# stecrotti/MPSKit.jl

Hardware: AMD Instinct MI355X
Metric: DMRG sweeps/sec + ddAC matvec achieved-TFLOP/s, Heisenberg L=100 D=1024 fp64 (higher is better)
Workload: dtype f64; 1 GPU; Heisenberg S=1/2 FiniteMPS L=100 D=1024 d=2 W=5 fp64, 1-site DMRG sweep (2L-2 site updates), fixed Krylov budget 8 matvecs/site; parallelism=single GPU

## Files before the change

include/mpsk.h:

```cpp
#ifndef MPSK_H
#define MPSK_H
#include <stddef.h>
#include <stdint.h>

#ifdef __cplusplus
extern "C" {
#endif

typedef struct mpsk_ctx mpsk_ctx;
typedef struct mpsk_mposlice mpsk_mposlice;

enum { MPSK_F64 = 0, MPSK_C128 = 1 };
enum { MPSK_OK = 0, MPSK_ERR_INVALID = 1, MPSK_ERR_HIP = 2, MPSK_ERR_UNSUPPORTED = 3, MPSK_ERR_NOMEM = 4 };
enum { MPSK_BLOCK_ZERO = 0, MPSK_BLOCK_SCALAR = 1, MPSK_BLOCK_DENSE = 2 };

int mpsk_version(void);
const char* mpsk_last_error(void);

int mpsk_ctx_create(int device, mpsk_ctx** out);
int mpsk_ctx_destroy(mpsk_ctx* ctx);
int mpsk_ctx_set_stream(mpsk_ctx* ctx, void* hip_stream);
int mpsk_ctx_set_dtype(mpsk_ctx* ctx, int dtype);
int mpsk_ctx_get_stream(mpsk_ctx* ctx, void** hip_stream);
int mpsk_ctx_get_device(mpsk_ctx* ctx, int* device);
// ... 39 lines not shown
int mpsk_hac_destroy(mpsk_hac* h);
int mpsk_hac_info(const mpsk_hac* h, int* mode, int* nslabs);
int mpsk_dC(mpsk_ctx* ctx, int W, int Dlo, int Dl, int Dr, const void* GL, const void* GR,
            const void* c, void* y);
int mpsk_dAC2(mpsk_ctx* ctx, const mpsk_mposlice* H1, const mpsk_mposlice* H2, int Dlo, int Dl, int Dr,
              const void* GL, const void* GR, const void* x2, void* y2);

int mpsk_dAC_proj(mpsk_ctx* ctx, const mpsk_mposlice* H, int Dlo, int Dl, int Dr, int Dro, const void* GL, const void* GR,
                  const void* x, void* y);
int mpsk_dAC2_proj(mpsk_ctx* ctx, const mpsk_mposlice* H1, const mpsk_mposlice* H2, int Dlo, int Dl, int Dm, int Dr, int Dro,
                   const void* GL, const void* GR, const void* AC, const void* AR, void* Y);

int mpsk_dAC2_product(mpsk_ctx* ctx, const mpsk_mposlice* H1, const mpsk_mposlice* H2, int Dl, int Dm, int Dr,
                      const void* GL, const void* GR, const void* AC, const void* AR, void* Y);
int mpsk_complement_tsvd(mpsk_ctx* ctx, int m, int n, const void* Y, int ldy, const void* QL, int ldql, int pl,
                         const void* QR, int ldqr, int pr, int k, void* U, int ldu, void* S, void* Vt, int ldvt, int* kept);
int mpsk_ctx_complement_stats(mpsk_ctx* ctx, long* n_calls, long* n_subspace, long* n_full);

int mpsk_transfer_left(mpsk_ctx* ctx, const mpsk_mposlice* H, int W, int d, int Dl, int Dr, int Dlb,
                       int Drb, const void* GLin, const void* A, const void* Ab, void* GLout);
int mpsk_transfer_right(mpsk_ctx* ctx, const mpsk_mposlice* H, int W, int d, int Dl, int Dr, int Dlb,
                        int Drb, const void* A, const void* Ab, const void* GRin, void* GRout);
enum { MPSK_TRANSFER_CANONICAL = 1 };
int mpsk_transfer_left_ex(mpsk_ctx* ctx, const mpsk_mposlice* H, int W, int d, int Dl, int Dr, int Dlb, int Drb,
                          const void* GLin, const void* A, const void* Ab, int flags, void* GLout);
int mpsk_transfer_right_ex(mpsk_ctx* ctx, const mpsk_mposlice* H, int W, int d, int Dl, int Dr, int Dlb, int Drb,
                           const void* A, const void* Ab, const void* GRin, int flags, void* GRout);
int mpsk_regularize(mpsk_ctx* ctx, int W, int D1, int D2, void* v, const void* lvec, const void* rvec);

int mpsk_qrpos(mpsk_ctx* ctx, int m, int n, const void* A, int lda, void* Q, int ldq, void* R, int ldr);
int mpsk_qrpos2(mpsk_ctx* ctx, int m, int n, const void* A1, int lda1, void* Q1, int ldq1, void* R1, int ldr1,
                const void* A2, int lda2, void* Q2, int ldq2, void* R2, int ldr2);
int mpsk_qrlq_pair(mpsk_ctx* ctx, int m, int n, const void* A1, int lda1, void* Q1, int ldq1, void* R1, int ldr1,
                   const void* A2, int lda2, void* L2, int ldl2, void* Q2, int ldq2);
int mpsk_lqpos(mpsk_ctx* ctx, int m, int n, const void* A, int lda, void* L, int ldl, void* Q, int ldq);
int mpsk_ctx_qr_defer(mpsk_ctx* ctx);
int mpsk_ctx_side_mark(mpsk_ctx* ctx);
int mpsk_ctx_side_begin(mpsk_ctx* ctx);
int mpsk_ctx_side_end(mpsk_ctx* ctx);
int mpsk_qr_commit(mpsk_ctx* ctx, int* redone);
int mpsk_tsvd(mpsk_ctx* ctx, int m, int n, const void* theta, int ldt, void* U, int ldu, void* S, void* Vh,
              int ldv, int max_keep, double trunc_err, int* kept, double* disc_norm);
int mpsk_tsplit(mpsk_ctx* ctx, int m, int n, const void* theta, int ldt, int max_keep, double trunc_err,
                void* AL, int ldal, void* C, int ldc, void* AR, int ldar, void* S, int* kept, double* disc_norm);
int mpsk_cx_embed(mpsk_ctx* ctx, int m, int n, const void* H, int64_t ldh, void* E, int64_t lde);
int mpsk_cx_half(mpsk_ctx* ctx, int m, int n, const void* E, int64_t lde, void* H, int64_t ldh);
// ... 40 lines not shown
```

mpskit.jl_amd/_lib.py:

```python
from __future__ import annotations

import ctypes as C
import os

_HERE = os.path.dirname(os.path.abspath(__file__))
LIB_PATH = os.environ.get("MPSK_LIB") or os.path.join(_HERE, "libmpsk.so")


class MpskError(RuntimeError):
    pass


_lib = None

c_void_pp = C.POINTER(C.c_void_p)
c_int32_p = C.POINTER(C.c_int32)
c_double_p = C.POINTER(C.c_double)

SIGNATURES = {
    "mpsk_ctx_create": [C.c_int, c_void_pp],
    "mpsk_ctx_destroy": [C.c_void_p],
    "mpsk_ctx_set_stream": [C.c_void_p, C.c_void_p],
    "mpsk_ctx_synchronize": [C.c_void_p],
    "mpsk_ctx_workspace_reserve": [C.c_void_p, C.c_size_t],
# ... 32 lines not shown
    "mpsk_dAC2": [C.c_void_p, C.c_void_p, C.c_void_p, C.c_int, C.c_int, C.c_int, C.c_void_p, C.c_void_p,
                  C.c_void_p, C.c_void_p],
    "mpsk_transfer_left": [C.c_void_p, C.c_void_p, C.c_int, C.c_int, C.c_int, C.c_int, C.c_int, C.c_int,
                           C.c_void_p, C.c_void_p, C.c_void_p, C.c_void_p],
    "mpsk_transfer_right": [C.c_void_p, C.c_void_p, C.c_int, C.c_int, C.c_int, C.c_int, C.c_int, C.c_int,
                            C.c_void_p, C.c_void_p, C.c_void_p, C.c_void_p],
    "mpsk_transfer_left_ex": [C.c_void_p, C.c_void_p, C.c_int, C.c_int, C.c_int, C.c_int, C.c_int, C.c_int,
                              C.c_void_p, C.c_void_p, C.c_void_p, C.c_int, C.c_void_p],
    "mpsk_transfer_right_ex": [C.c_void_p, C.c_void_p, C.c_int, C.c_int, C.c_int, C.c_int, C.c_int, C.c_int,
                               C.c_void_p, C.c_void_p, C.c_void_p, C.c_int, C.c_void_p],
    "mpsk_regularize": [C.c_void_p, C.c_int, C.c_int, C.c_int, C.c_void_p, C.c_void_p, C.c_void_p],
    "mpsk_qrpos": [C.c_void_p, C.c_int, C.c_int, C.c_void_p, C.c_int, C.c_void_p, C.c_int, C.c_void_p, C.c_int],
    "mpsk_qrpos2": [C.c_void_p, C.c_int, C.c_int, C.c_void_p, C.c_int, C.c_void_p, C.c_int, C.c_void_p, C.c_int,
                    C.c_void_p, C.c_int, C.c_void_p, C.c_int, C.c_void_p, C.c_int],
    "mpsk_qrlq_pair": [C.c_void_p, C.c_int, C.c_int, C.c_void_p, C.c_int, C.c_void_p, C.c_int, C.c_void_p, C.c_int,
                       C.c_void_p, C.c_int, C.c_void_p, C.c_int, C.c_void_p, C.c_int],
    "mpsk_lqpos": [C.c_void_p, C.c_int, C.c_int, C.c_void_p, C.c_int, C.c_void_p, C.c_int, C.c_void_p, C.c_int],
    "mpsk_tsvd": [C.c_void_p, C.c_int, C.c_int, C.c_void_p, C.c_int, C.c_void_p, C.c_int, C.c_void_p,
                  C.c_void_p, C.c_int, C.c_int, C.c_double, C.POINTER(C.c_int), c_double_p],
    "mpsk_tsplit": [C.c_void_p, C.c_int, C.c_int, C.c_void_p, C.c_int, C.c_int, C.c_double, C.c_void_p, C.c_int,
                    C.c_void_p, C.c_int, C.c_void_p, C.c_int, C.c_void_p, C.POINTER(C.c_int), c_double_p],
    "mpsk_gemm": [C.c_void_p, C.c_int, C.c_int, C.c_int, C.c_int, C.c_int, C.c_double, C.c_void_p,
                  C.c_int64, C.c_void_p, C.c_int64, C.c_double, C.c_void_p, C.c_int64],
    "mpsk_copy2d": [C.c_void_p, C.c_int, C.c_int, C.c_void_p, C.c_int64, C.c_void_p, C.c_int64],
    "mpsk_vdot": [C.c_void_p, C.c_int64, C.c_void_p, C.c_void_p, c_double_p],
    "mpsk_vnrm2": [C.c_void_p, C.c_int64, C.c_void_p, c_double_p],
    "mpsk_vaxpby": [C.c_void_p, C.c_int64, C.c_double, C.c_void_p, C.c_double, C.c_void_p],
    "mpsk_vscal": [C.c_void_p, C.c_int64, C.c_double, C.c_void_p],
    "mpsk_vtimes_i": [C.c_void_p, C.c_int64, C.c_void_p, C.c_void_p],
    "mpsk_vcopy": [C.c_void_p, C.c_int64, C.c_void_p, C.c_void_p],
    "mpsk_vzero": [C.c_void_p, C.c_int64, C.c_void_p],
    "mpsk_vmultidot": [C.c_void_p, C.c_int64, C.c_int, c_void_pp, C.c_void_p, c_double_p],
    "mpsk_vgs_step": [C.c_void_p, C.c_int64, C.c_int, c_void_pp, C.c_void_p, c_double_p],
    "mpsk_vorth_step": [C.c_void_p, C.c_int64, C.c_int, c_void_pp, C.c_void_p, c_double_p, c_double_p],
    "mpsk_vorth_step_dev": [C.c_void_p, C.c_int64, C.c_int, c_void_pp, C.c_void_p, C.c_void_p],
    "mpsk_vlincomb": [C.c_void_p, C.c_int64, C.c_int, c_void_pp, c_double_p, C.c_void_p],
    "mpsk_cx_embed": [C.c_void_p, C.c_int, C.c_int, C.c_void_p, C.c_int64, C.c_void_p, C.c_int64],
    "mpsk_cx_half": [C.c_void_p, C.c_int, C.c_int, C.c_void_p, C.c_int64, C.c_void_p, C.c_int64],
    "mpsk_vmultilincomb": [C.c_void_p, C.c_int64, C.c_int, c_void_pp, C.c_int, c_void_pp, c_double_p],
    "mpsk_vnormalize_dev": [C.c_void_p, C.c_int64, C.c_void_p, C.c_void_p, C.c_void_p],
    "mpsk_vnrm2_dev": [C.c_void_p, C.c_int64, C.c_void_p, C.c_void_p],
    "mpsk_ctx_qr_retries": [C.c_void_p, C.POINTER(C.c_long)],
    "mpsk_ctx_qr_defer": [C.c_void_p],
    "mpsk_ctx_side_mark": [C.c_void_p],
    "mpsk_ctx_side_begin": [C.c_void_p],
    "mpsk_ctx_side_end": [C.c_void_p],
# ... 96 lines not shown
```

mpskit.jl_amd/csrc/mpsk_api.hip:

```cpp
#include <hip/hip_runtime.h>
#include <cstdio>
#include <cstdlib>
#include <cstring>
#include <cmath>
#include <algorithm>
#include <map>
#include <string>
#include <vector>
#include "mpsk.h"
#include "mpsk_internal.h"

using namespace mpsk;

static thread_local std::string g_err;
static int fail(int code, const std::string& msg) { g_err = msg; return code; }
#define HIPCHK(expr)                                                                        \
  do {                                                                                      \
    hipError_t e_ = (expr);                                                                 \
    if (e_ != hipSuccess)                                                                   \
      return fail(MPSK_ERR_HIP, std::string(#expr) + ": " + hipGetErrorString(e_));         \
  } while (0)
#define REQUIRE(cond, msg)                                                  \
  do {                                                                      \
    if (!(cond)) return fail(MPSK_ERR_INVALID, std::string(__func__) + ": " + (msg)); \
  } while (0)

static constexpr int MPSK_DENSE_MIN_CHID = 8;

struct mpsk_mposlice {
  mpsk_ctx* ctx;
  int Wl, Wr, d;
  int dtype = MPSK_F64;
  std::vector<double> Ofull;
  std::vector<double> Ofull_im;
  MixPlan fwd;
  MixPlan bwd;
  MixPlan rgt;
  double Oi(int w, int t, int s, int v) const {
    return Ofull_im.empty() ? 0.0 : Ofull_im[w + (size_t)Wl * (t + d * (s + (size_t)d * v))];
  }
  std::vector<char> row_used, col_used;
  MixPlan rc;
  std::vector<int> rc_w, rc_s, rc_t;
  int rc_nseg = 0;
  bool jordan = false;
  MixPlan jr, jl;
  std::vector<int> jr_p, jl_p;
  int jr_nseg = 0, jl_nseg = 0;
  MixPlan tl, tr;
  bool tl_dblock = false;
  mutable std::map<int64_t, int64_t*> jtabL;
  mutable std::map<std::pair<int64_t, int64_t>, int64_t*> jtabR;
  double O(int w, int t, int s, int v) const { return Ofull[w + (size_t)Wl * (t + d * (s + (size_t)d * v))]; }
  bool dense = false;
  double* d_Od = nullptr;
  mutable std::map<std::pair<int64_t, int64_t>, int64_t*> dtab;
  double* d_OdR = nullptr;
  mutable std::map<std::pair<int64_t, int64_t>, int64_t*> dtabR;
};

struct PoolBuf { void* p; size_t bytes; bool used; hipStream_t last = nullptr; hipEvent_t ev = nullptr; bool ev_set = false; };

struct mpsk_ctx {
  int device = 0;
  hipStream_t stream = nullptr;
  void* ws = nullptr;
  size_t ws_bytes = 0;
  double* d_scal = nullptr;
  double* d_partial = nullptr;
  double* h_scal = nullptr;
  double* d_coef = nullptr;
  double* h_coef = nullptr;
  hipEvent_t ev_coef = nullptr;
// ... 347 lines not shown
        }
        out.assign((size_t)d * nseg, empty);
        for (int t = 0; t < d; ++t) {
          int k = 0;
          for (int si = 0; si < d; ++si) if (used[si + d * t]) out[(size_t)t * nseg + k++] = si + d * t;
        }
      };
      lists(r_used, s->jr_p, s->jr_nseg);
      lists(l_used, s->jl_p, s->jl_nseg);
      HIPCHK(mix_plan_create(jr, d * d, Wr, &s->jr));
      HIPCHK(mix_plan_create(jl, d * d, Wl, &s->jl));
      s->jordan = s->jr_nseg > 0 && s->jl_nseg > 0;
      if (s->jordan && !cx) {
        std::vector<MixTerm> tl, tr;
        for (int t = 0; t < d; ++t)
          for (int si = 0; si < d; ++si) {
            for (int v = 1; v < Wr; ++v)
              if (s->O(0, t, si, v) != 0.0) { tl.push_back({t + d * (v - 1), si, s->O(0, t, si, v)}); if (v == Wr - 1) s->tl_dblock = true; }
            for (int w = 1; w < Wl - 1; ++w)
              if (s->O(w, t, si, Wr - 1) != 0.0) tr.push_back({t + d * (w - 1), si, s->O(w, t, si, Wr - 1)});
          }
        HIPCHK(mix_plan_create(tl, d * (Wr - (s->tl_dblock ? 1 : 2)), d, &s->tl));
        HIPCHK(mix_plan_create(tr, d * (Wl - 2), d, &s->tr));
      }
    }
  }
  if (dense) {
    const int Wl = s->Wl, Wr = s->Wr;
    std::vector<double> od((size_t)d * Wl * d * Wr);
    for (int v = 0; v < Wr; ++v)
      for (int t = 0; t < d; ++t)
        for (int w = 0; w < Wl; ++w)
          for (int si = 0; si < d; ++si)
            od[(si + (size_t)d * w) + (size_t)d * Wl * (t + (size_t)d * v)] = s->O(w, t, si, v);
    s->dense = true;
    if (hipMalloc(&s->d_Od, sizeof(double) * od.size()) != hipSuccess) { mpsk_mposlice_destroy(s); return fail(MPSK_ERR_NOMEM, "dense MPO hipMalloc failed"); }
    HIPCHK(hipMemcpy(s->d_Od, od.data(), sizeof(double) * od.size(), hipMemcpyHostToDevice));
    for (int v = 0; v < Wr; ++v)
      for (int t = 0; t < d; ++t)
        for (int w = 0; w < Wl; ++w)
          for (int si = 0; si < d; ++si)
            od[(si + (size_t)d * v) + (size_t)d * Wr * (t + (size_t)d * w)] = s->O(w, t, si, v);
    if (hipMalloc(&s->d_OdR, sizeof(double) * od.size()) != hipSuccess) { mpsk_mposlice_destroy(s); return fail(MPSK_ERR_NOMEM, "dense MPO hipMalloc failed"); }
    HIPCHK(hipMemcpy(s->d_OdR, od.data(), sizeof(double) * od.size(), hipMemcpyHostToDevice));
  }
  *out = s;
// ... 15 lines not shown
  const void* blocks[1] = {O};
  return mposlice_build(c, dtype, 1, &cl, &cr, d, &kind, nullptr, blocks, true, out);
}

int mpsk_mposlice_destroy(mpsk_mposlice* s) {
  if (!s) return MPSK_OK;
  mpsk_ctx* c = s->ctx;
  (void)hipSetDevice(c->device);
  (void)hipStreamSynchronize(c->stream);
  for (auto it = c->pair_plans.begin(); it != c->pair_plans.end();) {
    if (it->first.first == s || it->first.second == s) { mix_plan_destroy(&it->second); it = c->pair_plans.erase(it); }
    else ++it;
  }
  mix_plan_destroy(&s->fwd);
  mix_plan_destroy(&s->bwd);
  mix_plan_destroy(&s->rgt);
  mix_plan_destroy(&s->rc);
  mix_plan_destroy(&s->jr);
  mix_plan_destroy(&s->jl);
  mix_plan_destroy(&s->tl);
  mix_plan_destroy(&s->tr);
  for (auto& kv : s->jtabL) (void)hipFree(kv.second);
  for (auto& kv : s->jtabR) (void)hipFree(kv.second);
  if (s->d_Od) (void)hipFree(s->d_Od);
  if (s->d_OdR) (void)hipFree(s->d_OdR);
  for (auto& kv : s->dtab) (void)hipFree(kv.second);
  for (auto& kv : s->dtabR) (void)hipFree(kv.second);
  delete s;
  return MPSK_OK;
}

int mpsk_mposlice_dims(const mpsk_mposlice* s, int* Wl, int* Wr, int* d) {
  REQUIRE(s, "slice is NULL");
  if (Wl) *Wl = s->Wl;
  if (Wr) *Wr = s->Wr;
  if (d) *d = s->d;
  return MPSK_OK;
}

}

static int ensure_ws(mpsk_ctx* c, size_t bytes) {
  if (c->pend.active) return fail(MPSK_ERR_INVALID, "a deferred factorization still owns the workspace: call mpsk_qr_commit first");
  if (c->on_side) return fail(MPSK_ERR_INVALID, "workspace users are not accepted on the side stream: call mpsk_ctx_side_end first");
  if (bytes <= c->ws_bytes) return MPSK_OK;
  return mpsk_ctx_workspace_reserve(c, bytes + bytes / 4);
}

static GemmArgs mk(const double* A, const double* B, double* C, int M, int N, int K, int64_t lda, int64_t ldb,
                   int64_t ldc, int tA = 0, int tB = 0) {
  GemmArgs g;
// ... 823 lines not shown
  if (left) { auto it = H->jtabL.find(Dl); if (it != H->jtabL.end()) { *out = it->second; return MPSK_OK; } }
  else { auto it = H->jtabR.find({Dl, Dr}); if (it != H->jtabR.end()) { *out = it->second; return MPSK_OK; } }
  const int d = H->d, n = left ? H->jl_nseg : H->jr_nseg;
  const std::vector<int>& plist = left ? H->jl_p : H->jr_p;
  const int64_t tL = (int64_t)Dl * d * Dl, tR = (int64_t)Dr * d * Dr;
  std::vector<int64_t> h((size_t)2 * d * n);
  for (int t = 0; t < d; ++t)
    for (int k = 0; k < n; ++k) {
      const int p = plist[(size_t)t * n + k], si = p % d, tt = p / d;
      if (left) { h[(size_t)t * n + k] = tt * tL + (int64_t)si * Dl; h[(size_t)(d + t) * n + k] = (int64_t)si * Dl; }
      else { h[(size_t)t * n + k] = (int64_t)si * Dl; h[(size_t)(d + t) * n + k] = tt * tR + (int64_t)si * Dr; }
    }
  int64_t* p = nullptr;
  if (hipMalloc(&p, sizeof(int64_t) * h.size()) != hipSuccess) return fail(MPSK_ERR_NOMEM, "transfer segment table hipMalloc failed");
  if (hipMemcpy(p, h.data(), sizeof(int64_t) * h.size(), hipMemcpyHostToDevice) != hipSuccess) {
    (void)hipFree(p);
    return fail(MPSK_ERR_HIP, "transfer segment table upload failed");
  }
  if (left) H->jtabL.emplace(Dl, p); else H->jtabR.emplace(std::make_pair((int64_t)Dl, (int64_t)Dr), p);
  *out = p;
  return MPSK_OK;
}

static int transfer_left_canonical(mpsk_ctx* c, const mpsk_mposlice* H, int Dl, int Dr, const double* GLin, const double* A,
                                   double* GLout) {
  const int d = H->d, Wr = H->Wr, n2 = H->jl_nseg;
  if (hac_check_on())
    if (int rc = transfer_canonical_check(c, "mpsk_transfer_left_ex", GLin, Dl, A, d, Dl, Dr, true)) return rc;
  const size_t slab = (size_t)Dl * d * Dr;
  const int64_t tL = (int64_t)Dl * d * Dl;
  const size_t nL = up32((size_t)d * tL);
  if (int rc = ensure_ws(c, sizeof(double) * (nL + slab * (Wr - 1)))) return rc;
  const int64_t* tab = nullptr;
  if (int rc = jordan_tab(H, true, Dl, Dr, &tab)) return rc;
  double* GLc = (double*)c->ws;
  double* T2 = GLc + nL;
  double* T = T2 + slab * (Wr - 2);
  SlabIndex il{1 << 30, 1, (int64_t)Dl * Dl, 0, 0, (int64_t)Dl}, ol{d, 1 << 30, (int64_t)Dl, tL, 0, (int64_t)d * Dl};
  HIPCHK(mix_apply(H->jl, GLin, il, GLc, ol, Dl, Dl, c->stream));
  SlabIndex ia{1 << 30, 1, (int64_t)Dl, 0, 0, (int64_t)Dl * d}, ot{d, 1 << 30, (int64_t)Dl, (int64_t)slab, 0, (int64_t)Dl * d};
  HIPCHK(mix_apply(H->tl, A, ia, T2, ot, Dl, Dr, c->stream));
  GemmArgs g = mk(GLc, A, T, Dl, Dr, Dl, (int64_t)Dl * d, (int64_t)Dl * d, (int64_t)Dl * d);
  g.batch = d; g.bsA = 0; g.bsB = 0; g.bsC = (int64_t)Dl;
  g.beta = H->tl_dblock ? 1.0 : 0.0;
  g.nseg = n2; g.zsegA = tab; g.zsegB = tab + (size_t)d * n2;
  g.tabs_even = Dl % 2 == 0;
  g.tag = 1;
  HIPCHK(gemm_f64(g, c->stream));
  HIPCHK(identity_slab(GLout, Dr, c->stream));
  GemmArgs g3 = mk(A, T2, GLout + (size_t)Dr * Dr, Dr, Dr, Dl * d, (int64_t)Dl * d, (int64_t)Dl * d, Dr, 1, 0);
  g3.batch = Wr - 1; g3.bsA = 0; g3.bsB = (int64_t)slab; g3.bsC = (int64_t)Dr * Dr;
  HIPCHK(gemm_f64(g3, c->stream));
  return MPSK_OK;
}

static int transfer_right_canonical(mpsk_ctx* c, const mpsk_mposlice* H, int Dl, int Dr, const double* A, const double* GRin,
                                    double* GRout) {
  const int d = H->d, Wl = H->Wl, Wr = H->Wr, n1 = H->jr_nseg;
  if (hac_check_on())
    if (int rc = transfer_canonical_check(c, "mpsk_transfer_right_ex", GRin + (size_t)(Wr - 1) * Dr * Dr, Dr, A, d, Dl, Dr, false))
      return rc;
  const size_t slab = (size_t)Dl * d * Dr;
  const int64_t tR = (int64_t)Dr * d * Dr;
  const size_t nR = up32((size_t)d * tR);
  if (int rc = ensure_ws(c, sizeof(double) * (nR + slab * (Wl - 1)))) return rc;
  const int64_t* tab = nullptr;
  if (int rc = jordan_tab(H, false, Dl, Dr, &tab)) return rc;
  double* GRc = (double*)c->ws;
  double* X = GRc + nR;
  SlabIndex ir{1 << 30, 1, (int64_t)Dr * Dr, 0, 0, (int64_t)Dr}, orr{d, 1 << 30, (int64_t)Dr, tR, 0, (int64_t)d * Dr};
  HIPCHK(mix_apply(H->jr, GRin, ir, GRc, orr, Dr, Dr, c->stream));
  SlabIndex ia{1 << 30, 1, (int64_t)Dl, 0, 0, (int64_t)Dl * d}, ox{d, 1 << 30, (int64_t)Dl, (int64_t)slab, 0, (int64_t)Dl * d};
  HIPCHK(mix_apply(H->tr, A, ia, X + slab, ox, Dl, Dr, c->stream));
  GemmArgs g = mk(A, GRc, X, Dl, Dr, Dr, (int64_t)Dl * d, (int64_t)Dr * d, (int64_t)Dl * d);
  g.batch = d; g.bsA = 0; g.bsB = 0; g.bsC = (int64_t)Dl;
  g.nseg = n1; g.zsegA = tab; g.zsegB = tab + (size_t)d * n1;
  g.tabs_even = Dl % 2 == 0 && Dr % 2 == 0;
  g.tag = 1;
  HIPCHK(gemm_f64(g, c->stream));
  HIPCHK(identity_slab(GRout + (size_t)(Wl - 1) * Dl * Dl, Dl, c->stream));
  std::vector<int64_t> sa;
  for (int t = 0; t < d; ++t) sa.push_back((int64_t)t * Dl);
  GemmArgs g3 = mk(X, A, GRout, Dl, Dl, Dr, (int64_t)Dl * d, (int64_t)Dl * d, Dl, 0, 1);
  g3.batch = Wl - 1; g3.bsA = (int64_t)slab; g3.bsB = 0; g3.bsC = (int64_t)Dl * Dl;
  HIPCHK(gemm_segments(g3, sa, sa, c->stream));
  return MPSK_OK;
}

int mpsk_transfer_left_ex(mpsk_ctx* c, const mpsk_mposlice* H, int W, int d, int Dl, int Dr, int Dlb, int Drb,
                          const void* GLin, const void* A, const void* Ab, int flags, void* GLout) {
  REQUIRE(c && GLin && A && Ab && GLout, "NULL argument");
  REQUIRE((flags & ~MPSK_TRANSFER_CANONICAL) == 0, "unknown flags");
  if (transfer_canonical_ok(H, flags, A, Ab, Dl, Dr, Dlb, Drb)) {
    REQUIRE(Dl > 0 && Dr > 0, "dimensions must be positive");
    HIPCHK(hipSetDevice(c->device));
    return transfer_left_canonical(c, H, Dl, Dr, (const double*)GLin, (const double*)A, (double*)GLout);
  }
  return mpsk_transfer_left(c, H, W, d, Dl, Dr, Dlb, Drb, GLin, A, Ab, GLout);
}

int mpsk_transfer_right_ex(mpsk_ctx* c, const mpsk_mposlice* H, int W, int d, int Dl, int Dr, int Dlb, int Drb,
                           const void* A, const void* Ab, const void* GRin, int flags, void* GRout) {
  REQUIRE(c && GRin && A && Ab && GRout, "NULL argument");
  REQUIRE((flags & ~MPSK_TRANSFER_CANONICAL) == 0, "unknown flags");
  if (transfer_canonical_ok(H, flags, A, Ab, Dl, Dr, Dlb, Drb)) {
    REQUIRE(Dl > 0 && Dr > 0, "dimensions must be positive");
    HIPCHK(hipSetDevice(c->device));
// ... 1710 lines not shown
```

mpskit.jl_amd/csrc/mpsk_gemm.hip:

```cpp
#include <hip/hip_runtime.h>
#include <stdint.h>
#include <cstdio>
#include <cstdlib>
#include <map>
#include <mutex>
#include <string>
#include <vector>
#include "mpsk_internal.h"

namespace mpsk {

typedef double d4 __attribute__((ext_vector_type(4)));
typedef double d2 __attribute__((ext_vector_type(2)));

constexpr int BK = 16;
constexpr int NTHREADS = 256;

template <int BMN, bool KMAJOR> struct LdsImg {
  static_assert(BK == 16, "the K-major swizzle assumes 128-byte rows");
  static constexpr int STRIDE = KMAJOR ? BK : (BMN + 16);
  static constexpr int SIZE = KMAJOR ? BMN * BK : BK * (BMN + 16);
  __device__ static inline int idx(int mn, int k) { return KMAJOR ? mn * BK + (k ^ (mn & 15)) : k * STRIDE + mn; }
};

// ... 378 lines not shown
  const int ntiles = tilesM * tilesN;
  int bid = blockIdx.x;
  if (!g.xcd_interleave) {
    int q = ntiles / 8, r = ntiles % 8, xcd = bid % 8, pos = bid / 8;
    bid = (xcd < r ? xcd * (q + 1) : r * (q + 1) + (xcd - r) * q) + pos;
  }
  int bm, bn;
  tile_coords(g, bid, tilesM, tilesN, &bm, &bn);
  if (g.upper_only && bm > bn) return;
  const int z = blockIdx.y;
  const int m0 = bm * BM, n0 = bn * BN;
  const double* Ab = g.A + (g.tabA ? g.tabA[z] : (int64_t)z * g.bsA);
  const double* Bb = g.B + (g.tabB ? g.tabB[z] : (int64_t)z * g.bsB);
  double* Cb = g.C + (g.tabC ? g.tabC[z] : (int64_t)z * g.bsC);
  d4 acc[BM / 32][BN / 32];
#pragma unroll
  for (int i = 0; i < BM / 32; ++i)
#pragma unroll
    for (int j = 0; j < BN / 32; ++j) acc[i][j] = d4{0.0, 0.0, 0.0, 0.0};
  const int nt = ((g.K + BK - 1) / BK) * g.nseg;
  int ktlo = 0, kthi = nt;
  if (g.b_upper) { const int lim = (n0 + BN + BK - 1) / BK; if (lim < kthi) kthi = lim; }
  if (g.a_upper) ktlo = m0 / BK;
  if (ktlo < kthi) gemm_acc_dispatch<BM, BN, TA, TB, ALIGNED, ZS, CJ>(g, Ab, Bb, z, m0, n0, ktlo, kthi, acc, smem);
  gemm_store_c<BM, BN, ALIGNED, CJ>(g, Cb, z, m0, n0, acc);
}

template <int BM, int BN, bool TA, bool TB, bool ALIGNED, bool ZS = false>
__device__ __forceinline__ void gemm_sk_body(const GemmArgs& g) {
  extern __shared__ __attribute__((aligned(16))) double smem[];
  constexpr int WTM = BM / 2, WTN = BN / 2, TM = WTM / 16, TN = WTN / 16;
  const int tilesM = (g.M + BM - 1) / BM, tilesN = (g.N + BN - 1) / BN;
  const int ntiles = tilesM * tilesN;
  const int KT = ((g.K + BK - 1) / BK) * g.nseg;
  const int U = ntiles * g.batch * KT;
  int sid = blockIdx.x;
  if (!g.xcd_interleave) {
    const int nwg = gridDim.x;
    int q = nwg / 8, r = nwg % 8, xcd = sid % 8, pos = sid / 8;
    sid = (xcd < r ? xcd * (q + 1) : r * (q + 1) + (xcd - r) * q) + pos;
  }
  int u = sid * g.sk_units;
  int slot = sid;
  if (g.sk_split_major) {
    const int TZ = ntiles * g.batch;
    const int split = sid / TZ, tzs = sid - split * TZ;
// ... 3 lines not shown
  const int uend = (u + g.sk_units < U) ? u + g.sk_units : U;
  const int lane = threadIdx.x & 63, wave = threadIdx.x >> 6;
  const int wm = wave & 1, wn = wave >> 1, fr = lane & 15, fq = lane >> 4;
  while (u < uend) {
    const int tz = u / KT;
    const int kt0 = u - tz * KT;
    const int kt1 = (uend - u < KT - kt0) ? kt0 + (uend - u) : KT;
    const int z = tz / ntiles, tile = tz - z * ntiles;
    int bm, bn;
    tile_coords(g, tile, tilesM, tilesN, &bm, &bn);
    if (g.upper_only && bm > bn) { u += kt1 - kt0; continue; }
    const int m0 = bm * BM, n0 = bn * BN;
    const double* Ab = g.A + (g.tabA ? g.tabA[z] : (int64_t)z * g.bsA);
    const double* Bb = g.B + (g.tabB ? g.tabB[z] : (int64_t)z * g.bsB);
    d4 acc[TM][TN];
#pragma unroll
    for (int i = 0; i < TM; ++i)
#pragma unroll
      for (int j = 0; j < TN; ++j) acc[i][j] = d4{0.0, 0.0, 0.0, 0.0};
    {
      int ka = kt0, kb = kt1;
      if (g.b_upper) { const int lim = (n0 + BN + BK - 1) / BK; if (lim < kb) kb = lim; }
      if (g.a_upper) { const int lo = m0 / BK; if (lo > ka) ka = lo; }
      if (ka < kb) gemm_acc_dispatch<BM, BN, TA, TB, ALIGNED, ZS, false>(g, Ab, Bb, z, m0, n0, ka, kb, acc, smem);
    }
    const bool toC = (kt0 == 0);
    double* base = toC ? g.C + (g.tabC ? g.tabC[z] : (int64_t)z * g.bsC) + m0 + (int64_t)n0 * g.ldc
                       : g.sk_ws + (int64_t)slot * BM * BN;
    const int64_t ld = toC ? g.ldc : BM;
    const double beta = toC ? g.beta : 0.0;
    const double alpha = g.alpha;
    const int mlim = toC ? g.M - m0 : BM, nlim = toC ? g.N - n0 : BN;
    const bool split = toC && g.tabC2 != nullptr;
#pragma unroll
    for (int i = 0; i < TM; ++i) {
      const int m = wm * WTM + i * 16 + fr;
#pragma unroll
      for (int j = 0; j < TN; ++j) {
#pragma unroll
        for (int rg = 0; rg < 4; ++rg) {
          const int n = wn * WTN + j * 16 + fq + 4 * rg;
          if (m < mlim && n < nlim) {
            double* p = base + m + (int64_t)n * ld;
            if (split && n0 + n >= g.splitN) p = g.C + g.tabC2[z] + (m0 + m) + (int64_t)(n0 + n - g.splitN) * g.ldc;
            double v = alpha * acc[i][j][rg];
            if (beta != 0.0) v += beta * (*p);
// ... 258 lines not shown
    if (--it->second.refs > 0) return;
    p = it->second.p;
    g_skws.erase(it);
  }
  if (p) { (void)hipStreamSynchronize(s); (void)hipFree(p); }
}

hipError_t gemm_f64(const GemmArgs& g_in, hipStream_t s) {
  GemmArgs g = g_in;
  if (g.M <= 0 || g.N <= 0 || g.batch <= 0) return hipSuccess;
  if (g.K <= 0 || g.nseg <= 0) {
    return hipErrorInvalidValue;
  }
  if (!g.A2 && !g.B2) { g.A2 = g.A; g.B2 = g.B; g.nseg1 = g.nseg; }
  else if (!g.A2 || !g.B2 || !g.zsegA || !g.zsegB || g.nseg1 < 0 || g.nseg1 > g.nseg) return hipErrorInvalidValue;
  int bm = 128, bn = 128;
  choose_tile(g.M, g.N, g.K * g.nseg, g.batch, &bm, &bn);
  g.sk_units = 0;
  g.sk_ws = nullptr;
  g.sk_split_major = 0;
  if (g.cplx && g.c_rs == 0) g.c_rs = 1;
  if (g.upper_only && g.M != g.N) g.upper_only = 0;
  if (g.nseg != 1 || g.transA || g.transB) g.a_upper = g.b_upper = 0;
  if (g_force_bm.load()) { bm = g_force_bm.load(); bn = g_force_bn.load(); }
  else if (g.cplx) {  }
  else {
    const int KT = ((g.K + BK - 1) / BK) * g.nseg;
    const int64_t Tb = (int64_t)((g.M + 127) / 128) * ((g.N + 127) / 128) * g.batch;
    const int64_t Ts = (int64_t)((g.M + 63) / 64) * ((g.N + 63) / 64) * g.batch;
    if (g_sk_enabled) {
      const int64_t Ub = Tb * KT;
      if (Tb >= 128 && Tb < 4 * 512 && Tb % 512 != 0 && Ub / 512 >= 16) {
        double* ws = sk_workspace(s);
        if (ws) { bm = bn = 128; g.sk_units = (int)((Ub + 511) / 512); g.sk_ws = ws; }
      }
    }
    if (g.sk_units == 0 && g_splitk_enabled && bm == 64 && bn == 64 && KT >= 64 && Ts <= 4096) {
      const int64_t slots = (int64_t)(SK_WS_DOUBLES / (64 * 64));
      int best_f = 1;
      double best = 0.0;
      for (int f = 1; f <= 8; ++f) {
        if (f > 1 && (KT / f < 16 || Ts * (f - 1) > slots)) break;
        const int64_t n = (Ts * f + 255) / 256;
        const int r = (int)(n % 4);
        const double phi[4] = {1.0, 0.55, 0.92, 0.98};
        const double len = (double)KT / f + 6.0;
// ... 264 lines not shown
```

mpskit.jl_amd/csrc/mpsk_internal.h:

```cpp
#pragma once
#include <hip/hip_runtime.h>
#include <stdint.h>
#include <stddef.h>
#include <atomic>
#include <vector>
#include <string>

namespace mpsk {

inline hipError_t ensure_dyn_smem(std::atomic<uint64_t>& done, const void* kernel, size_t bytes) {
  int dev = 0;
  hipError_t e = hipGetDevice(&dev);
  if (e != hipSuccess) return e;
  const uint64_t bit = 1ull << (dev & 63);
  if (done.load(std::memory_order_acquire) & bit) return hipSuccess;
  e = hipFuncSetAttribute(kernel, hipFuncAttributeMaxDynamicSharedMemorySize, (int)bytes);
  if (e != hipSuccess) return e;
  done.fetch_or(bit, std::memory_order_release);
  return hipSuccess;
}

constexpr int MAXSEG = 32;

struct GemmArgs {
// ... 10 lines not shown
  int transA, transB;
  const int64_t* tabA;
  const int64_t* tabB;
  const int64_t* tabC;
  const int64_t* tabC2;
  int splitN;
  int sk_units;
  int sk_split_major;
  double* sk_ws;
  int xcd_gx, xcd_gy;
  int xcd_interleave;
  const int64_t* zsegA;
  const int64_t* zsegB;
  const double* A2;
  const double* B2;
  int nseg1;
  signed char segJ[MAXSEG];
  int b_upper, a_upper;
  int upper_only;
  int cplx;
  int c_rs;
  int tag;
  int tabs_even;
};

hipError_t gemm_f64(const GemmArgs& g, hipStream_t s);
void gemm_force_tile(int bm, int bn);
void gemm_retain_stream(hipStream_t s);
void gemm_release_stream(hipStream_t s);
void gemm_enable_streamk(bool on);
void gemm_prof_enable(bool on);
std::string gemm_prof_summary();

struct GemmPairArgs {
  const double* P;
  const double* Q;
  const double* B;
  double* C1;
  double* C2;
  int M, N, K;
  int64_t ldp, ldq, ldb, ld1, ld2;
  const double* a1;
  const double* b1;
  const double* a2;
  const double* b2;
  double beta1, beta2;
};
hipError_t gemm_pair_f64(const GemmPairArgs& g, hipStream_t s);
hipError_t grassmann_coef(int K, const double* S, double scalar, int mode, double* coef, hipStream_t s);

struct MixTerm { int32_t out, in; double coef; double coef_im = 0.0; };

struct MixPlan {
  int n_out = 0, n_in = 0;
  int32_t* d_rowptr = nullptr;
  int32_t* d_src = nullptr;
  double* d_coef = nullptr;
  double* d_coef_im = nullptr;
  int nnz = 0;
  int max_terms = 0;
};

hipError_t mix_plan_create(const std::vector<MixTerm>& terms, int n_out, int n_in, MixPlan* plan);
void mix_plan_destroy(MixPlan* plan);

struct SlabIndex { int n0, n1; int64_t s0, s1, s2; int64_t ld; };
hipError_t mix_apply(const MixPlan& plan, const double* in, SlabIndex iin, double* out, SlabIndex iout,
                     int R, int C, hipStream_t s);
hipError_t deinterleave(const double* z, int64_t n, double* re, double* im, hipStream_t s);
hipError_t copy_strided(const double* src, int64_t srs, int64_t scs, double* dst, int64_t drs, int64_t dcs, int64_t R,
                        int64_t C, hipStream_t s);
hipError_t identity_slab(double* G, int n, hipStream_t s);

constexpr int MPSK_DOT_SCRATCH = 32 * 1024;
hipError_t vec_multidot(const double* const* xs, int k, const double* y, int64_t n, double* d_out,
                        double* d_partial, hipStream_t s);
hipError_t vec_diff_nrm2(const double* x, const double* y, int64_t n, double* d_out, double* d_partial, hipStream_t s);
hipError_t vec_axpby(double a, const double* x, double b, double* y, int64_t n, hipStream_t s);
hipError_t vec_times_i(const double* x, double* y, int64_t n, hipStream_t s);
hipError_t vec_scal(double a, double* x, int64_t n, hipStream_t s);
hipError_t vec_scal_rsqrt_dev(const double* d_n2, double* x, int64_t n, hipStream_t s);
hipError_t vec_scal_rsqrt_dev_oop(const double* d_n2, const double* x, double* y, int64_t n, hipStream_t s);
hipError_t vec_cgs2(const double* const* xs, int k, double* y, int64_t n, double* d_out, double* d_partial, hipStream_t s);
hipError_t vec_ritz_small(const double* d_slot, int m, int stride, double* d_coef, double* d_info, hipStream_t s);
hipError_t vec_multilincomb(const double* const* xs, int k, double* const* ys, int m, const double* d_coefs, int64_t n,
                            hipStream_t s);
hipError_t vec_multiaxpy(const double* const* xs, const double* d_coefs, int k, double sign, double* y,
                         int64_t n, hipStream_t s);
hipError_t vec_multidotc(const double* const* xs, int k, const double* y, int64_t n, double* d_out, double* d_partial,
                         hipStream_t s);
hipError_t vec_multiaxpy_c(const double* const* xs, const double* d_coefs, int k, double sign, double* y, int64_t n,
// ... 35 lines not shown
```

mpskit.jl_amd/csrc/mpsk_ops.hip:

```cpp
#include <hip/hip_runtime.h>
#include "mpsk_internal.h"

namespace mpsk {

typedef double d2 __attribute__((ext_vector_type(2)));

__device__ inline int64_t slab_off(const SlabIndex& ix, int j) {
  int j0 = j % ix.n0;
  int t = j / ix.n0;
  int j1 = t % ix.n1;
  int j2 = t / ix.n1;
  return j0 * ix.s0 + j1 * ix.s1 + j2 * ix.s2;
}

template <bool VEC2>
__global__ __launch_bounds__(256) void mix_kernel(const int32_t* __restrict__ rowptr,
                                                  const int32_t* __restrict__ src,
                                                  const double* __restrict__ coef,
                                                  const double* __restrict__ coef_im,
                                                  const double* __restrict__ in, SlabIndex iin,
                                                  double* __restrict__ out, SlabIndex iout, int R, int C) {
  const int o = blockIdx.y;
  const int t0 = rowptr[o], t1 = rowptr[o + 1];
  double* op = out + slab_off(iout, o);
  if (VEC2) {
    const int R2 = R >> 1;
    const int64_t total = (int64_t)R2 * C;
    for (int64_t e = blockIdx.x * (int64_t)blockDim.x + threadIdx.x; e < total;
         e += (int64_t)gridDim.x * blockDim.x) {
      int r = (int)(e % R2) * 2, c = (int)(e / R2);
      d2 acc = {0.0, 0.0};
      if (coef_im) {
        for (int t = t0; t < t1; ++t) {
          const double* ip = in + slab_off(iin, src[t]) + r + (int64_t)c * iin.ld;
          d2 v = *reinterpret_cast<const d2*>(ip);
          const double cr = coef[t], ci = coef_im[t];
          acc.x += cr * v.x - ci * v.y;
          acc.y += cr * v.y + ci * v.x;
        }
      } else {
        for (int t = t0; t < t1; ++t) {
          const double* ip = in + slab_off(iin, src[t]) + r + (int64_t)c * iin.ld;
          d2 v = *reinterpret_cast<const d2*>(ip);
          double cf = coef[t];
          acc.x += cf * v.x;
// ... 31 lines not shown
  if ((e = hipMalloc(&plan->d_src, sizeof(int32_t) * nz)) != hipSuccess) return e;
  if ((e = hipMalloc(&plan->d_coef, sizeof(double) * nz)) != hipSuccess) return e;
  if ((e = hipMemcpy(plan->d_rowptr, rowptr.data(), sizeof(int32_t) * (n_out + 1), hipMemcpyHostToDevice)) != hipSuccess) return e;
  if (terms.size()) {
    if ((e = hipMemcpy(plan->d_src, src.data(), sizeof(int32_t) * terms.size(), hipMemcpyHostToDevice)) != hipSuccess) return e;
    if ((e = hipMemcpy(plan->d_coef, coef.data(), sizeof(double) * terms.size(), hipMemcpyHostToDevice)) != hipSuccess) return e;
    if (cplx) {
      if ((e = hipMalloc(&plan->d_coef_im, sizeof(double) * nz)) != hipSuccess) return e;
      if ((e = hipMemcpy(plan->d_coef_im, coef_im.data(), sizeof(double) * terms.size(), hipMemcpyHostToDevice)) != hipSuccess) return e;
    }
  }
  return hipSuccess;
}

void mix_plan_destroy(MixPlan* plan) {
  if (plan->d_rowptr) (void)hipFree(plan->d_rowptr);
  if (plan->d_src) (void)hipFree(plan->d_src);
  if (plan->d_coef) (void)hipFree(plan->d_coef);
  if (plan->d_coef_im) (void)hipFree(plan->d_coef_im);
  *plan = MixPlan();
}

hipError_t mix_apply(const MixPlan& plan, const double* in, SlabIndex iin, double* out, SlabIndex iout,
                     int R, int C, hipStream_t s) {
  if (R <= 0 || C <= 0 || plan.n_out <= 0) return hipSuccess;
  bool vec2 = (R % 2 == 0) && (iin.ld % 2 == 0) && (iout.ld % 2 == 0) && (iin.s0 % 2 == 0) &&
              (iin.s1 % 2 == 0) && (iin.s2 % 2 == 0) && (iout.s0 % 2 == 0) && (iout.s1 % 2 == 0) &&
              (iout.s2 % 2 == 0) && ((uintptr_t)in % 16 == 0) && ((uintptr_t)out % 16 == 0);
  if (plan.d_coef_im && !vec2) return hipErrorInvalidValue;
  int64_t work = vec2 ? (int64_t)(R / 2) * C : (int64_t)R * C;
  int bx = (int)((work + 255) / 256);
  int cap = (2048 + plan.n_out - 1) / plan.n_out;
  if (cap < 1) cap = 1;
  if (bx > cap * 4) bx = cap * 4;
  if (bx < 1) bx = 1;
  dim3 grid(bx, plan.n_out, 1);
  if (vec2)
    hipLaunchKernelGGL(mix_kernel<true>, grid, dim3(256), 0, s, plan.d_rowptr, plan.d_src, plan.d_coef, plan.d_coef_im, in,
                       iin, out, iout, R, C);
  else
    hipLaunchKernelGGL(mix_kernel<false>, grid, dim3(256), 0, s, plan.d_rowptr, plan.d_src, plan.d_coef, plan.d_coef_im, in,
                       iin, out, iout, R, C);
  return hipGetLastError();
}

__global__ __launch_bounds__(256) void copy_strided_kernel(const double* __restrict__ src, int64_t srs, int64_t scs,
                                                           double* __restrict__ dst, int64_t drs, int64_t dcs, int64_t R,
                                                           int64_t C) {
  const int64_t total = R * C;
  for (int64_t e = blockIdx.x * (int64_t)blockDim.x + threadIdx.x; e < total; e += (int64_t)gridDim.x * blockDim.x) {
    const int64_t r = e % R, c = e / R;
    dst[r * drs + c * dcs] = src[r * srs + c * scs];
  }
}
__global__ __launch_bounds__(256) void deinterleave_kernel(const d2* __restrict__ z, double* __restrict__ re,
                                                           double* __restrict__ im, int64_t n) {
  for (int64_t e = blockIdx.x * (int64_t)blockDim.x + threadIdx.x; e < n; e += (int64_t)gridDim.x * blockDim.x) {
    const d2 v = z[e];
    re[e] = v.x;
    im[e] = v.y;
  }
}
hipError_t deinterleave(const double* z, int64_t n, double* re, double* im, hipStream_t s) {
  if (n <= 0) return hipSuccess;
  int64_t nb = (n + 255) / 256;
// ... 736 lines not shown
```

Before: 1.153 sweeps/s.

## Skip structurally-zero MPO blocks in canonical transfer mix and GEMM k-range

Builds a per-MPO-slice skip plan from the dense MPO tensor, finding for each virtual bond channel the contiguous range of physical indices that touch nonzero operator entries. The transfer mixing kernel then skips output slabs outside that range, and the transfer GEMMs clamp their k-tile range to it through a device table. This targets wasted FLOPs and memory traffic on zero operator blocks, such as Heisenberg S+/S- terms that connect only one physical index. It adds per-slice device tables, an environment switch, and guards against combination with segmented or complex GEMM.

```diff
diff --git a/include/mpsk.h b/include/mpsk.h
--- a/include/mpsk.h
+++ b/include/mpsk.h
@@ -85,6 +85,7 @@
 int mpsk_transfer_right(mpsk_ctx* ctx, const mpsk_mposlice* H, int W, int d, int Dl, int Dr, int Dlb,
                         int Drb, const void* A, const void* Ab, const void* GRin, void* GRout);
 enum { MPSK_TRANSFER_CANONICAL = 1 };
+int mpsk_zero_skip_plan(int Wl, int Wr, int d, const double* O, int left, int32_t* lo, int32_t* hi);
 int mpsk_transfer_left_ex(mpsk_ctx* ctx, const mpsk_mposlice* H, int W, int d, int Dl, int Dr, int Dlb, int Drb,
                           const void* GLin, const void* A, const void* Ab, int flags, void* GLout);
 int mpsk_transfer_right_ex(mpsk_ctx* ctx, const mpsk_mposlice* H, int W, int d, int Dl, int Dr, int Dlb, int Drb,
diff --git a/mpskit.jl_amd/_lib.py b/mpskit.jl_amd/_lib.py
--- a/mpskit.jl_amd/_lib.py
+++ b/mpskit.jl_amd/_lib.py
@@ -78,6 +78,7 @@
                     C.c_void_p, C.c_int, C.c_void_p, C.c_int, C.c_void_p, C.POINTER(C.c_int), c_double_p],
     "mpsk_gemm": [C.c_void_p, C.c_int, C.c_int, C.c_int, C.c_int, C.c_int, C.c_double, C.c_void_p,
                   C.c_int64, C.c_void_p, C.c_int64, C.c_double, C.c_void_p, C.c_int64],
+    "mpsk_zero_skip_plan": [C.c_int, C.c_int, C.c_int, C.c_void_p, C.c_int, C.c_void_p, C.c_void_p],
     "mpsk_copy2d": [C.c_void_p, C.c_int, C.c_int, C.c_void_p, C.c_int64, C.c_void_p, C.c_int64],
     "mpsk_vdot": [C.c_void_p, C.c_int64, C.c_void_p, C.c_void_p, c_double_p],
     "mpsk_vnrm2": [C.c_void_p, C.c_int64, C.c_void_p, c_double_p],
diff --git a/mpskit.jl_amd/csrc/mpsk_api.hip b/mpskit.jl_amd/csrc/mpsk_api.hip
--- a/mpskit.jl_amd/csrc/mpsk_api.hip
+++ b/mpskit.jl_amd/csrc/mpsk_api.hip
@@ -9,6 +9,7 @@
 #include <vector>
 #include "mpsk.h"
 #include "mpsk_internal.h"
+#include "mpsk_skip.h"
 
 using namespace mpsk;
 
@@ -49,6 +50,10 @@
   int jr_nseg = 0, jl_nseg = 0;
   MixPlan tl, tr;
   bool tl_dblock = false;
+  SkipPlan skl, skr;
+  unsigned char* d_tl_skip = nullptr;
+  unsigned char* d_tr_skip = nullptr;
+  mutable std::map<int64_t, int32_t*> zktL, zktR;
   mutable std::map<int64_t, int64_t*> jtabL;
   mutable std::map<std::pair<int64_t, int64_t>, int64_t*> jtabR;
   double O(int w, int t, int s, int v) const { return Ofull[w + (size_t)Wl * (t + d * (s + (size_t)d * v))]; }
@@ -442,6 +447,18 @@
           }
         HIPCHK(mix_plan_create(tl, d * (Wr - (s->tl_dblock ? 1 : 2)), d, &s->tl));
         HIPCHK(mix_plan_create(tr, d * (Wl - 2), d, &s->tr));
+        s->skl = skip_plan(s->Ofull.data(), Wl, Wr, d, true);
+        s->skr = skip_plan(s->Ofull.data(), Wl, Wr, d, false);
+        auto flags = [&](const SkipPlan& sk, int z0, int n_out, unsigned char** dev) -> int {
+          if (!sk.any || n_out <= 0) return MPSK_OK;
+          std::vector<unsigned char> f((size_t)n_out, 0);
+          for (int o = 0; o < n_out; ++o) { const int t = o % d, z = o / d + z0; f[o] = (t < sk.lo[z] || t >= sk.hi[z]) ? 1 : 0; }
+          if (hipMalloc(dev, f.size()) != hipSuccess) return fail(MPSK_ERR_NOMEM, "skip flags hipMalloc failed");
+          HIPCHK(hipMemcpy(*dev, f.data(), f.size(), hipMemcpyHostToDevice));
+          return MPSK_OK;
+        };
+        if (int rc = flags(s->skl, 0, s->tl.n_out, &s->d_tl_skip)) { mpsk_mposlice_destroy(s); return rc; }
+        if (int rc = flags(s->skr, 1, s->tr.n_out, &s->d_tr_skip)) { mpsk_mposlice_destroy(s); return rc; }
       }
     }
   }
@@ -503,11 +520,23 @@
   mix_plan_destroy(&s->tr);
   for (auto& kv : s->jtabL) (void)hipFree(kv.second);
   for (auto& kv : s->jtabR) (void)hipFree(kv.second);
+  for (auto& kv : s->zktL) (void)hipFree(kv.second);
+  for (auto& kv : s->zktR) (void)hipFree(kv.second);
+  if (s->d_tl_skip) (void)hipFree(s->d_tl_skip);
+  if (s->d_tr_skip) (void)hipFree(s->d_tr_skip);
   if (s->d_Od) (void)hipFree(s->d_Od);
   if (s->d_OdR) (void)hipFree(s->d_OdR);
   for (auto& kv : s->dtab) (void)hipFree(kv.second);
   for (auto& kv : s->dtabR) (void)hipFree(kv.second);
   delete s;
+  return MPSK_OK;
+}
+
+int mpsk_zero_skip_plan(int Wl, int Wr, int d, const double* O, int left, int32_t* lo, int32_t* hi) {
+  REQUIRE(O && lo && hi, "NULL argument");
+  REQUIRE(Wl >= 2 && Wr >= 2 && d > 0, "needs Wl, Wr >= 2 and d > 0");
+  const SkipPlan p = skip_plan(O, Wl, Wr, d, left != 0);
+  for (size_t z = 0; z < p.lo.size(); ++z) { lo[z] = p.lo[z]; hi[z] = p.hi[z]; }
   return MPSK_OK;
 }
 
@@ -1377,6 +1406,30 @@
   return MPSK_OK;
 }
 
+static bool zero_skip_on() { const char* ev = getenv("MPSK_ZERO_SKIP"); return !(ev && ev[0] == '0'); }
+
+static int skip_ktiles(const mpsk_mposlice* H, bool left, int D, const int32_t** out) {
+  *out = nullptr;
+  const SkipPlan& sk = left ? H->skl : H->skr;
+  if (!sk.any || !zero_skip_on() || H->d > MAXSEG) return MPSK_OK;
+  if (left && D % 16 != 0) return MPSK_OK;
+  auto& cache = left ? H->zktL : H->zktR;
+  auto it = cache.find(D);
+  if (it != cache.end()) { *out = it->second; return MPSK_OK; }
+  const int per = left ? D / 16 : (D + 15) / 16;
+  std::vector<int32_t> h(2 * sk.lo.size());
+  for (size_t z = 0; z < sk.lo.size(); ++z) { h[2 * z] = sk.lo[z] * per; h[2 * z + 1] = sk.hi[z] * per; }
+  int32_t* p = nullptr;
+  if (hipMalloc(&p, sizeof(int32_t) * h.size()) != hipSuccess) return fail(MPSK_ERR_NOMEM, "k-tile range table hipMalloc failed");
+  if (hipMemcpy(p, h.data(), sizeof(int32_t) * h.size(), hipMemcpyHostToDevice) != hipSuccess) {
+    (void)hipFree(p);
+    return fail(MPSK_ERR_HIP, "k-tile range table upload failed");
+  }
+  cache.emplace(D, p);
+  *out = p;
+  return MPSK_OK;
+}
+
 static int transfer_left_canonical(mpsk_ctx* c, const mpsk_mposlice* H, int Dl, int Dr, const double* GLin, const double* A,
                                    double* GLout) {
   const int d = H->d, Wr = H->Wr, n2 = H->jl_nseg;
@@ -1388,13 +1441,15 @@
   if (int rc = ensure_ws(c, sizeof(double) * (nL + slab * (Wr - 1)))) return rc;
   const int64_t* tab = nullptr;
   if (int rc = jordan_tab(H, true, Dl, Dr, &tab)) return rc;
+  const int32_t* zkt = nullptr;
+  if (int rc = skip_ktiles(H, true, Dl, &zkt)) return rc;
   double* GLc = (double*)c->ws;
   double* T2 = GLc + nL;
   double* T = T2 + slab * (Wr - 2);
   SlabIndex il{1 << 30, 1, (int64_t)Dl * Dl, 0, 0, (int64_t)Dl}, ol{d, 1 << 30, (int64_t)Dl, tL, 0, (int64_t)d * Dl};
   HIPCHK(mix_apply(H->jl, GLin, il, GLc, ol, Dl, Dl, c->stream));
   SlabIndex ia{1 << 30, 1, (int64_t)Dl, 0, 0, (int64_t)Dl * d}, ot{d, 1 << 30, (int64_t)Dl, (int64_t)slab, 0, (int64_t)Dl * d};
-  HIPCHK(mix_apply(H->tl, A, ia, T2, ot, Dl, Dr, c->stream));
+  HIPCHK(mix_apply(H->tl, A, ia, T2, ot, Dl, Dr, c->stream, zkt ? H->d_tl_skip : nullptr));
   GemmArgs g = mk(GLc, A, T, Dl, Dr, Dl, (int64_t)Dl * d, (int64_t)Dl * d, (int64_t)Dl * d);
   g.batch = d; g.bsA = 0; g.bsB = 0; g.bsC = (int64_t)Dl;
   g.beta = H->tl_dblock ? 1.0 : 0.0;
@@ -1405,6 +1460,7 @@
   HIPCHK(identity_slab(GLout, Dr, c->stream));
   GemmArgs g3 = mk(A, T2, GLout + (size_t)Dr * Dr, Dr, Dr, Dl * d, (int64_t)Dl * d, (int64_t)Dl * d, Dr, 1, 0);
   g3.batch = Wr - 1; g3.bsA = 0; g3.bsB = (int64_t)slab; g3.bsC = (int64_t)Dr * Dr;
+  g3.zkt = zkt;
   HIPCHK(gemm_f64(g3, c->stream));
   return MPSK_OK;
 }
@@ -1421,12 +1477,14 @@
   if (int rc = ensure_ws(c, sizeof(double) * (nR + slab * (Wl - 1)))) return rc;
   const int64_t* tab = nullptr;
   if (int rc = jordan_tab(H, false, Dl, Dr, &tab)) return rc;
+  const int32_t* zkt = nullptr;
+  if (int rc = skip_ktiles(H, false, Dr, &zkt)) return rc;
   double* GRc = (double*)c->ws;
   double* X = GRc + nR;
   SlabIndex ir{1 << 30, 1, (int64_t)Dr * Dr, 0, 0, (int64_t)Dr}, orr{d, 1 << 30, (int64_t)Dr, tR, 0, (int64_t)d * Dr};
   HIPCHK(mix_apply(H->jr, GRin, ir, GRc, orr, Dr, Dr, c->stream));
   SlabIndex ia{1 << 30, 1, (int64_t)Dl, 0, 0, (int64_t)Dl * d}, ox{d, 1 << 30, (int64_t)Dl, (int64_t)slab, 0, (int64_t)Dl * d};
-  HIPCHK(mix_apply(H->tr, A, ia, X + slab, ox, Dl, Dr, c->stream));
+  HIPCHK(mix_apply(H->tr, A, ia, X + slab, ox, Dl, Dr, c->stream, zkt ? H->d_tr_skip : nullptr));
   GemmArgs g = mk(A, GRc, X, Dl, Dr, Dr, (int64_t)Dl * d, (int64_t)Dr * d, (int64_t)Dl * d);
   g.batch = d; g.bsA = 0; g.bsB = 0; g.bsC = (int64_t)Dl;
   g.nseg = n1; g.zsegA = tab; g.zsegB = tab + (size_t)d * n1;
@@ -1438,6 +1496,7 @@
   for (int t = 0; t < d; ++t) sa.push_back((int64_t)t * Dl);
   GemmArgs g3 = mk(X, A, GRout, Dl, Dl, Dr, (int64_t)Dl * d, (int64_t)Dl * d, Dl, 0, 1);
   g3.batch = Wl - 1; g3.bsA = (int64_t)slab; g3.bsB = 0; g3.bsC = (int64_t)Dl * Dl;
+  g3.zkt = zkt;
   HIPCHK(gemm_segments(g3, sa, sa, c->stream));
   return MPSK_OK;
 }
diff --git a/mpskit.jl_amd/csrc/mpsk_gemm.hip b/mpskit.jl_amd/csrc/mpsk_gemm.hip
--- a/mpskit.jl_amd/csrc/mpsk_gemm.hip
+++ b/mpskit.jl_amd/csrc/mpsk_gemm.hip
@@ -424,6 +424,9 @@
   int ktlo = 0, kthi = nt;
   if (g.b_upper) { const int lim = (n0 + BN + BK - 1) / BK; if (lim < kthi) kthi = lim; }
   if (g.a_upper) ktlo = m0 / BK;
+  if constexpr (!ZS) {
+    if (g.zkt) { const int lo = g.zkt[2 * z], hi = g.zkt[2 * z + 1]; if (lo > ktlo) ktlo = lo; if (hi < kthi) kthi = hi; }
+  }
   if (ktlo < kthi) gemm_acc_dispatch<BM, BN, TA, TB, ALIGNED, ZS, CJ>(g, Ab, Bb, z, m0, n0, ktlo, kthi, acc, smem);
   gemm_store_c<BM, BN, ALIGNED, CJ>(g, Cb, z, m0, n0, acc);
 }
@@ -473,6 +476,9 @@
       int ka = kt0, kb = kt1;
       if (g.b_upper) { const int lim = (n0 + BN + BK - 1) / BK; if (lim < kb) kb = lim; }
       if (g.a_upper) { const int lo = m0 / BK; if (lo > ka) ka = lo; }
+      if constexpr (!ZS) {
+        if (g.zkt) { const int lo = g.zkt[2 * z], hi = g.zkt[2 * z + 1]; if (lo > ka) ka = lo; if (hi < kb) kb = hi; }
+      }
       if (ka < kb) gemm_acc_dispatch<BM, BN, TA, TB, ALIGNED, ZS, false>(g, Ab, Bb, z, m0, n0, ka, kb, acc, smem);
     }
     const bool toC = (kt0 == 0);
@@ -777,6 +783,7 @@
   if (g.cplx && g.c_rs == 0) g.c_rs = 1;
   if (g.upper_only && g.M != g.N) g.upper_only = 0;
   if (g.nseg != 1 || g.transA || g.transB) g.a_upper = g.b_upper = 0;
+  if (g.zkt && (g.zsegA || g.cplx)) return hipErrorInvalidValue;
   if (g_force_bm.load()) { bm = g_force_bm.load(); bn = g_force_bn.load(); }
   else if (g.cplx) {  }
   else {
diff --git a/mpskit.jl_amd/csrc/mpsk_internal.h b/mpskit.jl_amd/csrc/mpsk_internal.h
--- a/mpskit.jl_amd/csrc/mpsk_internal.h
+++ b/mpskit.jl_amd/csrc/mpsk_internal.h
@@ -56,6 +56,7 @@
   int c_rs;
   int tag;
   int tabs_even;
+  const int32_t* zkt;
 };
 
 hipError_t gemm_f64(const GemmArgs& g, hipStream_t s);
@@ -100,7 +101,7 @@
 
 struct SlabIndex { int n0, n1; int64_t s0, s1, s2; int64_t ld; };
 hipError_t mix_apply(const MixPlan& plan, const double* in, SlabIndex iin, double* out, SlabIndex iout,
-                     int R, int C, hipStream_t s);
+                     int R, int C, hipStream_t s, const unsigned char* d_skip = nullptr);
 hipError_t deinterleave(const double* z, int64_t n, double* re, double* im, hipStream_t s);
 hipError_t copy_strided(const double* src, int64_t srs, int64_t scs, double* dst, int64_t drs, int64_t dcs, int64_t R,
                         int64_t C, hipStream_t s);
diff --git a/mpskit.jl_amd/csrc/mpsk_ops.hip b/mpskit.jl_amd/csrc/mpsk_ops.hip
--- a/mpskit.jl_amd/csrc/mpsk_ops.hip
+++ b/mpskit.jl_amd/csrc/mpsk_ops.hip
@@ -19,8 +19,10 @@
                                                   const double* __restrict__ coef,
                                                   const double* __restrict__ coef_im,
                                                   const double* __restrict__ in, SlabIndex iin,
-                                                  double* __restrict__ out, SlabIndex iout, int R, int C) {
+                                                  double* __restrict__ out, SlabIndex iout, int R, int C,
+                                                  const unsigned char* __restrict__ skip) {
   const int o = blockIdx.y;
+  if (skip && skip[o]) return;
   const int t0 = rowptr[o], t1 = rowptr[o + 1];
   double* op = out + slab_off(iout, o);
   if (VEC2) {
@@ -98,7 +100,7 @@
 }
 
 hipError_t mix_apply(const MixPlan& plan, const double* in, SlabIndex iin, double* out, SlabIndex iout,
-                     int R, int C, hipStream_t s) {
+                     int R, int C, hipStream_t s, const unsigned char* d_skip) {
   if (R <= 0 || C <= 0 || plan.n_out <= 0) return hipSuccess;
   bool vec2 = (R % 2 == 0) && (iin.ld % 2 == 0) && (iout.ld % 2 == 0) && (iin.s0 % 2 == 0) &&
               (iin.s1 % 2 == 0) && (iin.s2 % 2 == 0) && (iout.s0 % 2 == 0) && (iout.s1 % 2 == 0) &&
@@ -113,10 +115,10 @@
   dim3 grid(bx, plan.n_out, 1);
   if (vec2)
     hipLaunchKernelGGL(mix_kernel<true>, grid, dim3(256), 0, s, plan.d_rowptr, plan.d_src, plan.d_coef, plan.d_coef_im, in,
-                       iin, out, iout, R, C);
+                       iin, out, iout, R, C, d_skip);
   else
     hipLaunchKernelGGL(mix_kernel<false>, grid, dim3(256), 0, s, plan.d_rowptr, plan.d_src, plan.d_coef, plan.d_coef_im, in,
-                       iin, out, iout, R, C);
+                       iin, out, iout, R, C, d_skip);
   return hipGetLastError();
 }
 
diff --git a/mpskit.jl_amd/csrc/mpsk_skip.h b/mpskit.jl_amd/csrc/mpsk_skip.h
--- /dev/null
+++ b/mpskit.jl_amd/csrc/mpsk_skip.h
@@ -0,0 +1,34 @@
+#pragma once
+#include <stddef.h>
+#include <vector>
+
+namespace mpsk {
+
+struct SkipPlan {
+  std::vector<int> lo, hi;
+  bool any = false;
+};
+
+inline SkipPlan skip_plan(const double* O, int Wl, int Wr, int d, bool left) {
+  SkipPlan p;
+  const int nb = (left ? Wr : Wl) - 1;
+  if (nb <= 0 || d <= 0) return p;
+  p.lo.assign(nb, 0);
+  p.hi.assign(nb, d);
+  auto at = [&](int w, int t, int s, int v) { return O[w + (size_t)Wl * (t + d * (s + (size_t)d * v))]; };
+  for (int z = 0; z < nb; ++z) {
+    if (left ? z == nb - 1 : z == 0) continue;
+    int lo = d, hi = 0;
+    for (int t = 0; t < d; ++t) {
+      bool used = false;
+      for (int s = 0; s < d && !used; ++s) used = (left ? at(0, t, s, z + 1) : at(z, t, s, Wr - 1)) != 0.0;
+      if (used) { if (t < lo) lo = t; hi = t + 1; }
+    }
+    if (hi == 0) lo = 0;
+    p.lo[z] = lo; p.hi[z] = hi;
+    if (lo != 0 || hi != d) p.any = true;
+  }
+  return p;
+}
+
+}
```

New measurement: 1.167 sweeps/s, median of 6. 1.2% higher.
